# nwihardjo/SpaghettiSearch

Measured on AMD Instinct MI355X. Metric: pagerank_iters_per_sec, higher is better.
Workload: dtype f64

## Files before the change

### spaghettisearch_amd/csrc/pagerank.hip

```cpp
#include "pr_device.hpp"

#include <algorithm>
#include <chrono>
#include <cmath>
#include <memory>

namespace {

__global__ void k_pr_item_ranges(WorkItem* __restrict__ work, uint32_t n_items, const uint32_t* __restrict__ in_ptr) {
    const uint32_t i = blockIdx.x * blockDim.x + threadIdx.x;
    if (i >= n_items) return;
    WorkItem w = work[i];
    switch (w.kind) {
        case V_ROWW: w.beg = in_ptr[w.row]; w.end = in_ptr[w.row + 1]; break;
        case V_SEG:
            w.beg = in_ptr[w.row] + w.count * SEGW;
            w.end = min(in_ptr[w.row + 1], w.beg + SEGW);
            break;
        case V_QUAD:
        case V_DEG: w.beg = in_ptr[w.row]; w.end = in_ptr[w.row + w.count]; break;
        default: return;
    }
    work[i] = w;
}
// ... 422 lines not shown
    if (!out) return ctx->fail(SS_ERR_INVALID, "ss_pr_create: out is NULL");
    *out = nullptr;
    if (k_topics < 1 || !n_topic) return ctx->fail(SS_ERR_INVALID, "ss_pr_create: k_topics < 1 or n_topic NULL");
    if (k_topics > MAXK) return ctx->fail(SS_ERR_UNSUPPORTED, "ss_pr_create: k_topics %d > %d per state (ss_pagerank_run splits larger K)", k_topics, MAXK);
    SS_HIP(ctx, hipSetDevice(ctx->device));
    hipStream_t st = ctx->stream;

    ss_pr* pr = new (std::nothrow) ss_pr();
    if (!pr) return ctx->fail(SS_ERR_OOM, "ss_pr_create: host OOM");
    std::unique_ptr<ss_pr> guard(pr);
    pr->g = g;
    pr->k = k_topics;
    pick_kernel(ctx, pr, k_topics, g->nd_int);
    const int GW = pr->gw;
    const bool vitems = pr->kernel != PR_STEP;
    const int GI = pr->nwave ? 8 : GW;
    const size_t n_local = g->n_local();
    if (((uint64_t)g->nd_int + 1) * GW * 8 >= (1ull << 32))
        return ctx->fail(SS_ERR_UNSUPPORTED, "ss_pr_create: contribution table of %llu rows x %d topics exceeds 4 GiB (shard the graph over more ranks)",
                         (unsigned long long)g->nd_int, GW);

    const bool trace = ctx->opt("pr.trace", 0) != 0;
    auto t_now = [] { return std::chrono::steady_clock::now(); };
    auto t_ms = [](std::chrono::steady_clock::time_point a, std::chrono::steady_clock::time_point b) { return std::chrono::duration<double, std::milli>(b - a).count(); };
    SS_HIP(ctx, pr->x.alloc(n_local * GW));
    bool share = GW >= 8 && g->world == 1 && ctx->opt("pr.affine", 0) == 0 && ctx->opt("pr.share_zero_rows", 1) != 0;
    if (!share) SS_TRY(alloc_tables(pr, st, (size_t)g->nd_int + 1));

    const auto tc0 = t_now();
    const PlanOptions opt = plan_options(ctx, pr, n_local);
    Cut cut = cut_items(g->h_indeg_nd, g->h_indeg_d, g->sl_nd, GI, pr->nwave, opt);
    const uint32_t n_tail = g->cnt_nd - cut.pos_nd;
    struct PinGuard { ss_ctx* c; void* p = nullptr; size_t cap = 0; ~PinGuard() { c->pin_free(p, cap); } } tail_od{ctx};
    if (share && n_tail == 0) {
        share = false;
        SS_TRY(alloc_tables(pr, st, (size_t)g->nd_int + 1));
    }
    if (share) {
        tail_od.p = ctx->pin_alloc((size_t)n_tail * sizeof(uint32_t), &tail_od.cap);
        if (!tail_od.p) return ctx->fail(SS_ERR_OOM, "ss_pr_create: no pinned host memory for %u out-degrees", n_tail);
        SS_HIP(ctx, hipMemcpyAsync(tail_od.p, g->outdeg.p + cut.pos_nd, (size_t)n_tail * sizeof(uint32_t), hipMemcpyDeviceToHost, st));
    }
    const auto tc1 = t_now();
    const int per_cu = blocks_per_cu(pr->kernel, GW);
    const auto tc1a = t_now();
    pr->nblocks = grid_for(ctx, pr, opt, per_cu, cut.items.size());
    static const std::vector<uint32_t> no_woff;
    const std::vector<uint32_t>* woff = &no_woff;
    if (vitems) {
        const uint32_t nw = pr->nblocks * WAVES;
        const auto td0 = t_now();
        const std::vector<double>& cost = item_costs(cut, g->h_indeg_nd, g->h_indeg_d, g->sl_nd, GI, pr->nwave);
        const auto td0a = t_now();
        std::vector<uint32_t>& owner = deal_items(cut, cost, nw, pr->nwave, opt);
#ifdef SS_PR_WAVETIME
        dump_wave_loads(cut, cost, owner, nw);
#endif
        const auto td1 = t_now();
        if (trace) fprintf(stderr, "[pr trace]   deal: occupancy query %.2f ms, costs %.3f ms, owners %.3f ms\n", t_ms(tc1, tc1a), t_ms(td0, td0a), t_ms(td0a, td1));
        woff = &place_items(cut, owner, nw);
        if (trace) fprintf(stderr, "[pr trace]   deal: placement %.3f ms\n", t_ms(td1, t_now()));
    }
    const std::vector<WorkItem>& items = cut.items;

    g->settle();
    const auto tc2 = t_now();
    SharedRows sh;
    if (share) {
        SS_HIP(ctx, hipStreamSynchronize(st));
        const auto ts0 = t_now();
        sh = plan_shared_rows(static_cast<const uint32_t*>(tail_od.p), n_tail, cut.pos_nd);
        const auto ts1 = t_now();
        SS_TRY(alloc_tables(pr, st, (size_t)sh.table_rows));
        SS_HIP(ctx, pr->sh_deg.alloc(sh.deg.size()));
        SS_HIP(ctx, hipMemcpyAsync(pr->sh_deg.p, sh.deg.data(), sh.deg.size() * sizeof(uint32_t), hipMemcpyHostToDevice, st));
        SS_HIP(ctx, pr->src_shared.alloc(g->e_local));
        if (g->e_local)
            hipLaunchKernelGGL(k_pr_remap_src, dim3((unsigned)std::min<uint64_t>(ss::div_up(g->e_local, TPB), (uint64_t)ctx->cu_count * 16)), dim3(TPB), 0, st,
                               (const uint32_t*)g->in_src.p, pr->src_shared.p, (size_t)g->e_local, cut.pos_nd, g->cnt_nd, (const uint32_t*)g->outdeg.p,
                               (const uint32_t*)pr->sh_deg.p, (uint32_t)sh.deg.size(), sh.zrow);
        if (trace) fprintf(stderr, "[pr trace]   shared rows: %u rows without in-edges -> %zu shared rows (host %.3f ms), table %llu rows\n", n_tail, sh.deg.size(),
                           t_ms(ts0, ts1), (unsigned long long)sh.table_rows);
    }
    SS_HIP(ctx, pr->partials.alloc(((size_t)std::max(pr->nblocks, ss::begin_blocks(pr)) + 8) * 2 * GW));
    SS_HIP(ctx, pr->segpart.alloc((size_t)std::max(cut.nsegs, 1u) * GW));
    SS_HIP(ctx, pr->rowticket.alloc(std::max(cut.nmulti, 1u)));
    SS_HIP(ctx, hipMemsetAsync(pr->rowticket.p, 0, pr->rowticket.bytes(), st));
    SS_HIP(ctx, pr->woff.alloc(std::max<size_t>(woff->size(), 8)));
    if (!woff->empty()) SS_HIP(ctx, hipMemcpyAsync(pr->woff.p, woff->data(), woff->size() * sizeof(uint32_t), hipMemcpyHostToDevice, st));
    SS_HIP(ctx, pr->work.alloc(items.size()));
    SS_HIP(ctx, hipMemcpyAsync(pr->work.p, items.data(), items.size() * sizeof(WorkItem), hipMemcpyHostToDevice, st));
    if (vitems)
        hipLaunchKernelGGL(k_pr_item_ranges, dim3(ss::div_up(items.size(), TPB)), dim3(TPB), 0, st, pr->work.p, (uint32_t)items.size(), (const uint32_t*)g->in_ptr.p);
    SS_HIP(ctx, pr->ctl.alloc(1));
    SS_HIP(ctx, hipMemsetAsync(pr->ctl.p, 0, sizeof(PrCtl), st));
    double h_x0[MAXK];
    for (int k = 0; k < MAXK; k++) h_x0[k] = k < k_topics ? 1.0 / (double)n_topic[k] : 0.0;
    SS_HIP(ctx, pr->x0.alloc(MAXK));
    SS_HIP(ctx, hipMemcpyAsync(pr->x0.p, h_x0, sizeof(h_x0), hipMemcpyHostToDevice, st));
    SS_HIP(ctx, hipStreamSynchronize(st));
    if (trace) fprintf(stderr, "[pr trace] ss_pr_create: build_work %.2f ms (%zu items), edge ranges + deal %.2f ms, alloc + upload %.2f ms\n", t_ms(tc0, tc1), items.size(), t_ms(tc1, tc2), t_ms(tc2, t_now()));
    if (trace) fprintf(stderr, "[pr trace] where the state lives: x %p  tab0 %p  tab1 %p  in_src %p  in_ptr %p  outdeg %p  work %p  woff %p\n", (void*)pr->x.p, (void*)pr->tab0.p,
                       (void*)pr->tab1.p, (void*)g->in_src.p, (void*)g->in_ptr.p, (void*)g->outdeg.p, (void*)pr->work.p, (void*)pr->woff.p);

    fill_params(pr, cut, opt, damping, eps, max_iter, k_topics);
    if (share) {
        PrParams& p = pr->prm;
        p.in_src = pr->src_shared.p;
        p.sh_deg = pr->sh_deg.p;
        p.n_shared = (uint32_t)sh.deg.size();
        p.share = 1;
        p.zrow = sh.zrow;
        p.tab_rows = cut.pos_nd;
    }
    if (trace) trace_plan(pr, items, *woff);
    g->users++;
    *out = guard.release();
    return SS_OK;
}

int32_t ss_pr_set_teleport(ss_pr* pr, const uint64_t* set_ptr, const uint32_t* set_nodes) {
    if (!pr) return SS_ERR_INVALID;
    ss_ctx* ctx = pr->g->ctx;
    std::lock_guard<std::recursive_mutex> lk(ctx->mu);
    SS_HIP(ctx, hipSetDevice(ctx->device));
    if (pr->begun) return ctx->fail(SS_ERR_STATE, "ss_pr_set_teleport: call before ss_pr_begin");
    hipStream_t st = ctx->stream;
    PrParams& p = pr->prm;
    if (!set_ptr) {
        p.memb = nullptr; p.tin = nullptr; p.nz_in = nullptr; p.ts_mask = 0;
        return SS_OK;
    }
    const ss_graph* g = pr->g;
    const int K = pr->k;
    SS_TRY(unshare_rows(pr, st));
    std::vector<uint64_t> h_ptr(K + 1);
    SS_HIP(ctx, ss::copy_in(ctx->stream, h_ptr.data(), set_ptr, (K + 1) * sizeof(uint64_t)));
    if (h_ptr[0] != 0) return ctx->fail(SS_ERR_INVALID, "ss_pr_set_teleport: set_ptr[0] != 0");
    for (int k = 0; k < K; k++)
        if (h_ptr[k + 1] < h_ptr[k]) return ctx->fail(SS_ERR_INVALID, "ss_pr_set_teleport: set_ptr not non-decreasing");
    const uint64_t total = h_ptr[K];
    if (total && !set_nodes) return ctx->fail(SS_ERR_INVALID, "ss_pr_set_teleport: set_nodes is NULL");
    double h_tin[MAXK];
    uint32_t mask = 0;
    for (int k = 0; k < MAXK; k++) {
        h_tin[k] = 0.0;
        if (k < K && h_ptr[k + 1] > h_ptr[k]) {
            mask |= 1u << k;
            h_tin[k] = p.teleport * (double)g->n / (double)(h_ptr[k + 1] - h_ptr[k]);
        }
    }
    const size_t n_local = g->n_local();
    ss::DevBuf<uint64_t> d_ptr;
    ss::DevBuf<uint32_t> d_nodes, d_err, d_seen;
    ss::DevBuf<unsigned long long> d_cnt;
    SS_HIP(ctx, d_ptr.alloc(K + 1));
    SS_HIP(ctx, d_seen.alloc(g->n));
    SS_HIP(ctx, hipMemsetAsync(d_seen.p, 0, std::max<size_t>(d_seen.bytes(), 4), st));
    SS_HIP(ctx, d_nodes.alloc(total));
    SS_HIP(ctx, d_err.alloc(1));
    SS_HIP(ctx, d_cnt.alloc(MAXK));
    SS_HIP(ctx, pr->memb.alloc(n_local));
    SS_HIP(ctx, pr->tin.alloc(MAXK));
    SS_HIP(ctx, pr->nz_in.alloc(MAXK));
    SS_HIP(ctx, hipMemcpyAsync(d_ptr.p, h_ptr.data(), (K + 1) * sizeof(uint64_t), hipMemcpyHostToDevice, st));
    if (total) SS_HIP(ctx, hipMemcpyAsync(d_nodes.p, set_nodes, total * sizeof(uint32_t), hipMemcpyDefault, st));
    SS_HIP(ctx, hipMemsetAsync(pr->memb.p, 0, std::max<size_t>(pr->memb.bytes(), 4), st));
// ... 245 lines not shown
```

### spaghettisearch_amd/csrc/pr_device.hpp

```cpp
#pragma once
#include "pr_state.hpp"

#include <cmath>

namespace {


template <int GW>
__device__ __forceinline__ double wave_sum_topic(double v) {
#pragma unroll
    for (int off = GW; off < 64; off <<= 1) v += __shfl_xor(v, off, 64);
    return v;
}

__device__ __forceinline__ double zero_row_rank(const PrParams& p, int sweep, double S, double x0) {
    return ((sweep == 0 ? x0 : 0.0) + p.teleport) / S;
}
__device__ __forceinline__ double teleport_of(const PrParams& p, uint32_t lrow, int t) {
    if (!p.memb || !((p.ts_mask >> t) & 1u)) return p.teleport;
    return ((p.memb[lrow] >> t) & 1u) ? p.tin[t] : 0.0;
}
__device__ __forceinline__ double zero_row_rank_ts(const PrParams& p, int sweep, double S, double x0, double tele) {
    return ((sweep == 0 ? x0 : 0.0) + tele) / S;
}

template <int PS, typename T>
__device__ __forceinline__ T ctl_ld(const T* q) {
    if constexpr (PS) return __hip_atomic_load(q, __ATOMIC_RELAXED, __HIP_MEMORY_SCOPE_AGENT);
    else return *q;
}
template <int PS, typename T>
__device__ __forceinline__ void ctl_st(T* q, T v) {
    if constexpr (PS) __hip_atomic_store(q, v, __ATOMIC_RELAXED, __HIP_MEMORY_SCOPE_AGENT);
    else *q = v;
}

template <int PS = 0>
__device__ __forceinline__ void finalize_ctl(const PrParams& p, const double* dl, const double* cs, bool is_begin) {
    PrCtl* ctl = p.ctl;
    if (p.aff) {
        AffCtl* a = p.aff;
        if (is_begin) {
            const double r1 = cs[0], s1 = cs[1] + p.tele_n, sigma = r1 + s1;
            for (int k = 0; k < MAXK; k++) {
                const bool real = k < 2;
                ctl->xz[k] = real ? p.x0[k] : 0.0;
                ctl->xz_in[k] = ctl->xz[k];
                ctl->S[k] = real ? sigma : 1.0;
                ctl->csum[k] = real ? cs[k] : 0.0;
                ctl->delta[k] = 0.0;
                ctl->active[k] = real ? 1 : 0;
                ctl->iters[k] = 0;
                ctl->tele[k] = 0.0;
            }
            ctl->tele[1] = p.teleport;
            a->r_x = 0.0; a->s_x = 1.0;
            a->r_prev = 0.0; a->s_prev = 1.0;
            a->r_next = r1 / sigma; a->s_next = s1 / sigma;
            a->xz_prev[0] = ctl->xz[0];
            a->xz_prev[1] = ctl->xz[1];
            a->it = 0;
            ctl->sweep = 0;
            ctl->n_active = 2;
            return;
        }
        const int it = ctl->sweep + 1;
        a->r_prev = a->r_x; a->s_prev = a->s_x;
        a->r_x = a->r_next; a->s_x = a->s_next;
        for (int k = 0; k < 2; k++) {
            a->xz_prev[k] = ctl->xz[k];
            ctl->xz[k] = zero_row_rank_ts(p, ctl->sweep, ctl->S[k], p.x0[k], ctl->tele[k]);
            ctl->xz_in[k] = ctl->xz[k];
            ctl->iters[k] = it;
            ctl->csum[k] = cs[k];
        }
        const double r1 = cs[0] + p.tele_n * a->r_x;
        const double s1 = cs[1] + p.tele_n * a->s_x;
        const double sigma = r1 + s1;
        a->r_next = r1 / sigma;
        a->s_next = s1 / sigma;
        ctl->tele[0] = p.teleport * a->r_x;
        ctl->tele[1] = p.teleport * a->s_x;
        ctl->S[0] = ctl->S[1] = sigma;
        ctl->sweep = it;
        return;
    }
    if (is_begin) {
        for (int k = 0; k < MAXK; k++) {
            const bool real = k < p.k_topics;
            ctl->xz[k] = real ? p.x0[k] : 0.0;
            ctl->xz_in[k] = real ? p.x0[k] : 0.0;
            ctl->S[k] = real ? cs[k] + p.tele_n : 1.0;
            ctl->csum[k] = real ? cs[k] : 0.0;
            ctl->delta[k] = 0.0;
            ctl->active[k] = real ? 1 : 0;
            ctl->iters[k] = 0;
        }
        ctl->sweep = 0;
        ctl->n_active = p.k_topics;
        return;
    }
    const int sw = ctl_ld<PS>(&ctl->sweep);
    const int it = sw + 1;
    int na = 0;
    for (int k = 0; k < p.k_topics; k++) {
        if (ctl_ld<PS>(&ctl->active[k])) {
            const double Sk = ctl_ld<PS>(&ctl->S[k]);
            ctl_st<PS>(&ctl->iters[k], it);
            ctl_st<PS>(&ctl->delta[k], dl[k]);
            if (p.memb && ((p.ts_mask >> k) & 1u)) {
                ctl_st<PS>(&ctl->xz[k], zero_row_rank_ts(p, sw, Sk, p.x0[k], 0.0));
                ctl_st<PS>(&ctl->xz_in[k], zero_row_rank_ts(p, sw, Sk, p.x0[k], p.tin[k]));
            } else {
                const double xz = zero_row_rank(p, sw, Sk, p.x0[k]);
                ctl_st<PS>(&ctl->xz[k], xz);
                ctl_st<PS>(&ctl->xz_in[k], xz);
            }
            bool cont = dl[k] > p.eps;
            if (p.max_iter > 0 && it >= p.max_iter) cont = false;
            ctl_st<PS>(&ctl->active[k], cont ? 1 : 0);
            na += cont ? 1 : 0;
            ctl_st<PS>(&ctl->S[k], cs[k] + p.tele_n);
            ctl_st<PS>(&ctl->csum[k], cs[k]);
        }
    }
    ctl_st<PS>(&ctl->n_active, na);
    if constexpr (PS) {
        asm volatile("s_waitcnt vmcnt(0)" ::: "memory");
    }
    ctl_st<PS>(&ctl->sweep, it);
}

template <int GW, int PS = 0>
__device__ __forceinline__ void block_reduce_and_publish(const PrParams& p, double dsum, double csum, double* tail,
                                                         bool is_begin) {
    __shared__ double red[WAVES][2][MAXK];
    __shared__ double tot[2][MAXK];
    __shared__ double colsum[TPB];
    __shared__ int s_last;
    const int lane = threadIdx.x & 63, wave = threadIdx.x >> 6;
    const int t = lane % GW;
    dsum = wave_sum_topic<GW>(dsum);
    csum = wave_sum_topic<GW>(csum);
    if (lane < GW) {
        red[wave][0][t] = dsum;
        red[wave][1][t] = csum;
    }
    __syncthreads();
    if (threadIdx.x < 2 * GW) {
        const int which = threadIdx.x / GW, tt = threadIdx.x % GW;
        double v = red[0][which][tt];
#pragma unroll
        for (int w = 1; w < WAVES; w++) v += red[w][which][tt];
        __hip_atomic_store(&p.partials[(size_t)blockIdx.x * 2 * GW + threadIdx.x], v, __ATOMIC_RELAXED, __HIP_MEMORY_SCOPE_AGENT);
    }
    asm volatile("s_waitcnt vmcnt(0)" ::: "memory");
    __syncthreads();
    constexpr unsigned NG = 8;
    constexpr int NCOL = 2 * GW;
    constexpr int NPART = TPB / NCOL;
    const unsigned ng = min(NG, gridDim.x);
    const unsigned grp = blockIdx.x % ng;
    const unsigned members = (gridDim.x - grp + ng - 1) / ng;
    double* const gpart = p.partials + (size_t)gridDim.x * NCOL;
    if (threadIdx.x == 0) {
        if constexpr (PS == 2) {
            __builtin_amdgcn_fence(__ATOMIC_RELEASE, "agent");
            asm volatile("s_waitcnt vmcnt(0)" ::: "memory");
        }
        const unsigned prev = __hip_atomic_fetch_add(&p.ctl->gticket[grp], 1u, __ATOMIC_RELAXED, __HIP_MEMORY_SCOPE_AGENT);
        s_last = prev == members - 1;
    }
    __syncthreads();
    if (!s_last) return;
    const int col = threadIdx.x % NCOL, part = threadIdx.x / NCOL;
    {
        double acc = 0.0;
        for (unsigned m0 = part; m0 < members; m0 += 16 * NPART) {
            double v[16];
#pragma unroll
            for (int u = 0; u < 16; u++) {
                const unsigned m = m0 + u * NPART;
                v[u] = __hip_atomic_load(&p.partials[(size_t)(grp + ng * (m < members ? m : m0)) * NCOL + col], __ATOMIC_RELAXED, __HIP_MEMORY_SCOPE_AGENT);
            }
#pragma unroll
            for (int u = 0; u < 16; u++)
                if (m0 + u * NPART < members) acc += v[u];
        }
        colsum[threadIdx.x] = acc;
    }
    __syncthreads();
    if (threadIdx.x < NCOL) {
        double v = 0.0;
        for (int q = 0; q < NPART; q++) v += colsum[q * NCOL + threadIdx.x];
        __hip_atomic_store(&gpart[(size_t)grp * NCOL + threadIdx.x], v, __ATOMIC_RELAXED, __HIP_MEMORY_SCOPE_AGENT);
    }
    if (threadIdx.x == 0) ctl_st<PS>(&p.ctl->gticket[grp], 0u);
    asm volatile("s_waitcnt vmcnt(0)" ::: "memory");
    __syncthreads();
    if (threadIdx.x == 0) {
        const unsigned prev = __hip_atomic_fetch_add(&p.ctl->ticket, 1u, __ATOMIC_RELAXED, __HIP_MEMORY_SCOPE_AGENT);
        s_last = prev == ng - 1;
    }
    __syncthreads();
    if (!s_last) return;
    if (threadIdx.x < NCOL) {
        double v = 0.0;
        for (unsigned gq = 0; gq < ng; gq++)
            v += __hip_atomic_load(&gpart[(size_t)gq * NCOL + threadIdx.x], __ATOMIC_RELAXED, __HIP_MEMORY_SCOPE_AGENT);
        tot[threadIdx.x / GW][threadIdx.x % GW] = v;
    }
    __syncthreads();
    if (!is_begin && threadIdx.x < GW && ctl_ld<PS>(&p.ctl->active[threadIdx.x])) {
        const double n_zero = (double)((p.cnt_nd - p.pos_nd) + (p.cnt_d - p.pos_d));
        if (p.memb && ((p.ts_mask >> threadIdx.x) & 1u)) {
            const int k = threadIdx.x;
            const double out_new = zero_row_rank_ts(p, ctl_ld<PS>(&p.ctl->sweep), ctl_ld<PS>(&p.ctl->S[k]), p.x0[k], 0.0);
            const double in_new = zero_row_rank_ts(p, ctl_ld<PS>(&p.ctl->sweep), ctl_ld<PS>(&p.ctl->S[k]), p.x0[k], p.tin[k]);
            tot[0][k] += (n_zero - p.nz_in[k]) * fabs(out_new - ctl_ld<PS>(&p.ctl->xz[k])) + p.nz_in[k] * fabs(in_new - ctl_ld<PS>(&p.ctl->xz_in[k]));
        } else {
            const double xz_new = zero_row_rank(p, ctl_ld<PS>(&p.ctl->sweep), ctl_ld<PS>(&p.ctl->S[threadIdx.x]), p.x0[threadIdx.x]);
            tot[0][threadIdx.x] += n_zero * fabs(xz_new - ctl_ld<PS>(&p.ctl->xz[threadIdx.x]));
        }
    }
    __syncthreads();
    if (p.world == 1) {
        if (threadIdx.x == 0) {
            double dl[MAXK], cs[MAXK];
            for (int k = 0; k < MAXK; k++) {
                dl[k] = k < GW ? tot[0][k] : 0.0;
                cs[k] = k < GW ? tot[1][k] : 0.0;
            }
            ctl_st<PS>(&p.ctl->ticket, 0u);
            finalize_ctl<PS>(p, dl, cs, is_begin);
        }
    } else {
        if (threadIdx.x < GW) {
            tail[(size_t)(p.sl_nd - 2) * GW + threadIdx.x] = tot[1][threadIdx.x];
            tail[(size_t)(p.sl_nd - 1) * GW + threadIdx.x] = tot[0][threadIdx.x];
        }
        if (threadIdx.x == 0) p.ctl->ticket = 0;
    }
}

template <int GA, int GB>
__device__ __attribute__((used, noinline)) void begin_caller_context(const PrParams& p, double* tail) {
    if (!__builtin_constant_p(p.world)) return;
    block_reduce_and_publish<GA>(p, 0.0, 0.0, tail, true);
    block_reduce_and_publish<GB>(p, 0.0, 0.0, tail, true);
}

#define NT_LOAD(p) __builtin_nontemporal_load(p)
#define NT_STORE(v, p) __builtin_nontemporal_store(v, p)

constexpr uint32_t SRC_MASK = 0x7FFFFFFFu;

}
```

### spaghettisearch_amd/csrc/pr_state.hpp

```cpp
#pragma once
#include "graph.hpp"
#include "pr_plan.hpp"

#ifdef SS_PR_WAVETIME
#include <cstdio>
#include <cstdlib>
#include <string>
#endif

namespace {

constexpr int MAXK = 16;

struct PrCtl {
    double S[MAXK];
    double delta[MAXK];
    double csum[MAXK];
    double xz[MAXK];
    double xz_in[MAXK];
    double tele[MAXK];
    int32_t active[MAXK];
    int32_t iters[MAXK];
    int32_t sweep;
    int32_t n_active;
    uint32_t ticket;
    uint32_t stuck;
    uint32_t gticket[8];
};

constexpr int AFF_MAXK = 256;
constexpr unsigned AFF_NB = 512;
struct AffCtl {
    double u[AFF_MAXK];
    double delta[AFF_MAXK];
    int32_t active[AFF_MAXK], iters[AFF_MAXK], just[AFF_MAXK];
    double r_x, r_prev, r_next;
    double s_x, s_prev, s_next;
    double xz_prev[2];
    int32_t n_active, n_just, k_real, it;
};

struct PrParams {
    const uint32_t* in_ptr;
    const uint32_t* in_src;
    const uint32_t* outdeg;
    double* x;
    const double* tab_rd[2];
    double* tab_wr[2];
    const WorkItem* work;
    double* partials;
    double* segpart;
    uint32_t* rowticket;
    PrCtl* ctl;
    const double* x0;
    double d, teleport, eps, tele_n;
    int32_t max_iter, k_topics, world;
    uint32_t sl_nd, cnt_nd, sl_d, cnt_d, seg_edges, n_items;
    uint32_t pos_nd, pos_d;
    const uint32_t* memb;
    const double* tin;
    const double* nz_in;
    uint32_t ts_mask;
    uint32_t zrow;
    const uint32_t* woff;
    uint32_t stagger_div;
    uint32_t stagger_code;
    uint32_t class_order;
    uint32_t n_order;
    double* x_alt;
    AffCtl* aff;
    const double* tele_col;
    const uint32_t* sh_deg;
    uint32_t n_shared;
    uint32_t share;
    uint32_t tab_rows;
};

}

enum PrKernel : int {
    PR_STEP = 0,
    PR_SWEEP = 1,
    PR_SWEEP_N = 2,
};

struct ss_pr {
    ss_graph* g = nullptr;
    PrKernel kernel = PR_SWEEP;
    int gw = 1;
    ss::DevBuf<float> wire_send, wire_recv;
    bool nwave = false;
    int persist_mode = 1;
    bool persist = false;
    int k = 1;
    PrParams prm{};
    unsigned nblocks = 0;
    ss::DevBuf<double> x, tab0, tab1, send, partials, segpart, x0;
    ss::DevBuf<uint32_t> rowticket;
    ss::DevBuf<uint32_t> memb;
    ss::DevBuf<double> tin, nz_in;
    ss::DevBuf<WorkItem> work;
    ss::DevBuf<uint32_t> woff;
    ss::DevBuf<uint32_t> src_shared;
    ss::DevBuf<uint32_t> sh_deg;
    ss::DevBuf<PrCtl> ctl;
    bool begun = false;
    bool need_finalize = false;
    bool finalize_is_begin = false;
};

// ... 41 lines not shown
```

### spaghettisearch_amd/csrc/pr_sweep.hip

```cpp
#include "pr_device.hpp"

#include <algorithm>

namespace {

template <int GW>
__device__ __forceinline__ double tab_at(const double* __restrict__ T, uint32_t row, int t) {
    return *reinterpret_cast<const double*>(reinterpret_cast<const char*>(T) + (size_t)((row * (uint32_t)GW + (uint32_t)t) * 8u));
}


template <int GW, bool TS>
struct SweepCtx {
    const PrParams& p;
    const double* __restrict__ T;
    double* __restrict__ Tw;
    double S, x0;
    bool act;
    int t, gbase, slot;
    double dsum, csum;
};

__device__ __forceinline__ uint32_t turn_fill(uint32_t epos, uint32_t lim) {
    return min((uint32_t)CH, __builtin_elementwise_sub_sat(lim, epos));
// ... 150 lines not shown
        for (int j = 0; j < CH; j++) acc += v[j];
        if (ends) {
            const uint32_t od = (uint32_t)__shfl((int)co, c.gbase + (int)q, 64);
            if (valid) finish_row<GW>(c, lrow, acc, xo, od);
            acc = 0.0;
        }
        q = qn;
        ch = cn;
        if (cross) {
            it++;
            cur = nxt;
            cb = nb; ce = ne; co = no;
            nq = (cur.count + NS - 1) / NS;
            nch = cur.nseg;
            nxt = work[it + 1];
            bounds(nxt, it + 1 < i1, nb, ne, no);
        }
    }
}

template <int GW, int R, bool TS>
__device__ __forceinline__ void deg_rows(SweepCtx<GW, TS>& c, const WorkItem* __restrict__ work, uint32_t i0, uint32_t i1) {
    constexpr int NS = 64 / GW;
    constexpr int DM = CH / R;
    constexpr int IR = CH / GW;
    const PrParams& p = c.p;
    if (i0 >= i1) return;
    auto idx = [&](const WorkItem& w, bool live, uint32_t turn, uint32_t (&src)[IR]) __attribute__((always_inline)) {
        const uint32_t rb = (turn * NS + (uint32_t)c.slot) * R;
#pragma unroll
        for (int r = 0; r < IR; r++) {
            const uint32_t j = (uint32_t)(r * GW + c.t);
            const uint32_t rr = rb + j / DM, u = j % DM;
            const bool ok = live && u < w.nseg && rr < w.count;
            const uint32_t raw = NT_LOAD(&p.in_src[ok ? w.beg + rr * w.nseg + u : 0u]);
            src[r] = ok ? (raw & SRC_MASK) : p.zrow;
        }
    };
    WorkItem cur = work[i0], nxt = work[i0 + 1];
    uint32_t src_n[IR];
    idx(cur, true, 0, src_n);
    for (uint32_t it = i0; it < i1; it++) {
        const WorkItem nn = work[it + 2];
        const uint32_t row0 = cur.row, count = cur.count;
        const uint32_t turns = (count + NS * R - 1) / (NS * R);
        for (uint32_t i = 0; i < turns; i++) {
            uint32_t src[IR];
#pragma unroll
            for (int r = 0; r < IR; r++) src[r] = src_n[r];
            if (i + 1 < turns) idx(cur, true, i + 1, src_n);
            else idx(nxt, it + 1 < i1, 0, src_n);
            const uint32_t rb = (i * NS + (uint32_t)c.slot) * R;
            double xo[R];
#pragma unroll
            for (int r = 0; r < R; r++) xo[r] = NT_LOAD(&p.x[(size_t)(row0 + (rb + r < count ? rb + r : 0u)) * GW + c.t]);
            const uint32_t myr = row0 + (rb + (uint32_t)c.t < count ? rb + (uint32_t)c.t : 0u);
            const uint32_t odv = (c.t < R && myr < p.sl_nd) ? NT_LOAD(&p.outdeg[myr]) : 1u;
            double v[CH];
            gather_turn<GW>(c.T, src, c.t, c.gbase, v);
#pragma unroll
            for (int r = 0; r < R; r++) {
                double y = 0.0;
#pragma unroll
                for (int u = 0; u < DM; u++) y += v[r * DM + u];
                const uint32_t od = (uint32_t)__shfl((int)odv, c.gbase + r, 64);
                if (rb + r < count) finish_row<GW>(c, row0 + rb + r, y, xo[r], od);
            }
        }
        cur = nxt;
        nxt = nn;
    }
}

#ifndef SS_PR_MINW
#define SS_PR_MINW 1
#endif
#ifdef SS_PR_WAVETIME
__device__ unsigned long long g_pr_wt[65536][2];
#endif
template <int GW, bool TS>
__global__ __launch_bounds__(TPB, SS_PR_MINW) void k_pr_sweep(PrParams p) {
    constexpr int NS = 64 / GW;
    PrCtl* ctl = p.ctl;
    if (ctl->n_active == 0) return;
#ifdef SS_PR_WAVETIME
    unsigned long long wt0;
    asm volatile("s_memrealtime %0\n\ts_waitcnt lgkmcnt(0)" : "=s"(wt0));
#endif
    const int sweep = ctl->sweep;
    const int lane = threadIdx.x & 63;
    const uint32_t wave = (uint32_t)__builtin_amdgcn_readfirstlane((int)(threadIdx.x >> 6));
    SweepCtx<GW, TS> c{p, p.tab_rd[sweep & 1], p.tab_wr[sweep & 1], 0.0, 0.0, false, lane % GW, lane - lane % GW, lane / GW, 0.0, 0.0};
    c.S = ctl->S[c.t];
    c.act = ctl->active[c.t] != 0;
    c.x0 = sweep == 0 ? p.x0[c.t] : 0.0;

    if constexpr (!TS) {
        if (p.n_shared) {
            const double xz_out = c.act ? zero_row_rank(p, sweep, c.S, p.x0[c.t]) : ctl->xz[c.t];
            const uint32_t nel = p.n_shared * (uint32_t)GW;
            for (uint32_t i = blockIdx.x * TPB + threadIdx.x; i < nel; i += gridDim.x * TPB)
                c.Tw[(size_t)(p.zrow + 1) * GW + i] = p.d * xz_out / (double)p.sh_deg[i / GW];
        }
    }

    const uint32_t* __restrict__ off = p.woff + (size_t)(blockIdx.x * WAVES + wave) * 8;
    int rot = p.stagger_div ? (int)((blockIdx.x / p.stagger_div) % 6u) : 0;
    if (p.stagger_code) {
        uint32_t cdv = p.stagger_code;
        for (uint32_t r = blockIdx.x / p.stagger_div; r > 0; r--) cdv /= 6u;
        rot = (int)(cdv % 6u);
    }
    for (int s6 = 0; s6 < 6; s6++) {
    const int cls = (int)((p.class_order >> (3 * ((s6 + rot) % 6))) & 7u);
    {
        int ln = lane;
        asm volatile("" : "+v"(ln));
        c.t = ln % GW;
        c.gbase = ln - ln % GW;
        c.slot = ln / GW;
    }
    switch (cls) {
    case 0: long_rows<GW>(c, p.work, off[0], off[1], lane); break;
    case 1: quad_rows<GW>(c, p.work, off[1], off[2]); break;
    case 2: deg_rows<GW, 2>(c, p.work, off[2], off[3]); break;
    case 3: deg_rows<GW, 4>(c, p.work, off[3], off[4]); break;
    case 4: deg_rows<GW, 8>(c, p.work, off[4], off[5]); break;
    default:
    for (uint32_t item = off[5]; item < off[6]; item++) {
        const WorkItem w = p.work[item];
        const bool store = TS || !p.share;
        const bool ts = TS && p.memb && ((p.ts_mask >> c.t) & 1u);
        const double xz_out = c.act ? (ts ? zero_row_rank_ts(p, sweep, c.S, p.x0[c.t], 0.0) : zero_row_rank(p, sweep, c.S, p.x0[c.t])) : ctl->xz[c.t];
        const double xz_inn = ts ? (c.act ? zero_row_rank_ts(p, sweep, c.S, p.x0[c.t], p.tin[c.t]) : ctl->xz_in[c.t]) : xz_out;
        uint32_t od[16];
#pragma unroll
        for (int i = 0; i < 16; i++) {
            const uint32_t rr = (uint32_t)(i * NS + c.slot);
            od[i] = NT_LOAD(&p.outdeg[w.row + (rr < w.count ? rr : 0u)]);
        }
#pragma unroll
        for (int i = 0; i < 16; i++) {
            const uint32_t rr = (uint32_t)(i * NS + c.slot);
            if (rr < w.count) {
                const uint32_t lrow = w.row + rr;
                const double xz = ts && ((p.memb[lrow] >> c.t) & 1u) ? xz_inn : xz_out;
                const double cc = p.d * xz / (double)od[i];
                if (store) NT_STORE(cc, &c.Tw[(size_t)lrow * GW + c.t]);
                c.csum += cc;
            }
        }
    }
    break;
    }
    }
#ifdef SS_PR_WAVETIME
    {
        unsigned long long wt1;
        asm volatile("s_waitcnt vmcnt(0)\n\ts_memrealtime %0\n\ts_waitcnt lgkmcnt(0)" : "=s"(wt1));
        const uint32_t wid = (blockIdx.x * WAVES + wave) & 65535u;
        if (lane == 0) { g_pr_wt[wid][0] = wt0; g_pr_wt[wid][1] = wt1; }
    }
#endif
    block_reduce_and_publish<GW>(p, c.dsum, c.csum, c.Tw, false);
}

template __device__ void begin_caller_context<8, 16>(const PrParams&, double*);

}

namespace ss {
void pr_sweep_launch(ss_pr* pr, hipStream_t st) {
    const bool ts = pr->prm.memb != nullptr;
    if (pr->gw == 8) {
        if (ts) hipLaunchKernelGGL((k_pr_sweep<8, true>), dim3(pr->nblocks), dim3(TPB), 0, st, pr->prm);
        else hipLaunchKernelGGL((k_pr_sweep<8, false>), dim3(pr->nblocks), dim3(TPB), 0, st, pr->prm);
    } else {
        if (ts) hipLaunchKernelGGL((k_pr_sweep<16, true>), dim3(pr->nblocks), dim3(TPB), 0, st, pr->prm);
        else hipLaunchKernelGGL((k_pr_sweep<16, false>), dim3(pr->nblocks), dim3(TPB), 0, st, pr->prm);
    }
}
int pr_sweep_occupancy(int gw) {
    int per_cu = 8;
    if (gw == 8) (void)hipOccupancyMaxActiveBlocksPerMultiprocessor(&per_cu, k_pr_sweep<8, false>, TPB, 0);
    else (void)hipOccupancyMaxActiveBlocksPerMultiprocessor(&per_cu, k_pr_sweep<16, false>, TPB, 0);
    return per_cu;
}

#ifdef SS_PR_WAVETIME
void pr_dump_wave_times(const ss_pr* pr) {
    if (pr->gw < 8) return;
    (void)hipDeviceSynchronize();
    const uint32_t nwv = std::min<uint32_t>(65536u, pr->nblocks * WAVES);
    std::vector<unsigned long long> h((size_t)nwv * 2);
    if (hipMemcpyFromSymbol(h.data(), HIP_SYMBOL(g_pr_wt), h.size() * sizeof(unsigned long long)) != hipSuccess || !nwv) return;
    unsigned long long t0 = ~0ull;
    for (uint32_t w = 0; w < nwv; w++) t0 = std::min(t0, h[2 * w]);
    std::vector<double> st(nwv), en(nwv);
    for (uint32_t w = 0; w < nwv; w++) { st[w] = (double)(h[2 * w] - t0) / 100.0; en[w] = (double)(h[2 * w + 1] - t0) / 100.0; }
    std::sort(st.begin(), st.end()); std::sort(en.begin(), en.end());
    if (FILE* f = open_dump("pr_wt.csv")) {
        fprintf(f, "wave,start_us,end_us\n");
        for (uint32_t w = 0; w < nwv; w++) fprintf(f, "%u,%.2f,%.2f\n", w, (double)(h[2 * w] - t0) / 100.0, (double)(h[2 * w + 1] - t0) / 100.0);
        fclose(f);
    }
    fprintf(stderr, "[pr wavetime] %u waves: start us median %.1f max %.1f | out of items us min %.1f p10 %.1f median %.1f p90 %.1f p99 %.1f max %.1f\n", nwv,
            st[nwv / 2], st[nwv - 1], en[0], en[nwv / 10], en[nwv / 2], en[nwv * 9 / 10], en[(size_t)nwv * 99 / 100], en[nwv - 1]);
}
#endif
}
```

### spaghettisearch_amd/csrc/pr_sweep_n.hip

```cpp
#include "pr_device.hpp"

namespace {

#ifndef SS_PRN_MINW
#define SS_PRN_MINW 6
#endif
template <int KW>
struct NVec { double v[KW]; };
template <int KW, int PS = 0>
__device__ __forceinline__ NVec<KW> ntab(const double* __restrict__ T, uint32_t row) {
    NVec<KW> r;
    if constexpr (PS == 1) {
        const double* q = reinterpret_cast<const double*>(reinterpret_cast<const char*>(T) + (size_t)(row * (8u * KW)));
#pragma unroll
        for (int k = 0; k < KW; k++) r.v[k] = __hip_atomic_load(q + k, __ATOMIC_RELAXED, __HIP_MEMORY_SCOPE_AGENT);
    } else if constexpr (KW == 1) {
        r.v[0] = *reinterpret_cast<const double*>(reinterpret_cast<const char*>(T) + (size_t)(row * 8u));
    } else {
        const double2 t = *reinterpret_cast<const double2*>(reinterpret_cast<const char*>(T) + (size_t)(row * 16u));
        r.v[0] = t.x;
        r.v[1] = t.y;
    }
    return r;
}
// ... 187 lines not shown
    #pragma unroll
                        for (int u = 0; u < 4; u++) {
                            const uint32_t j = b + ch * 16u + (uint32_t)(u * 8 + gl);
                            const uint32_t raw = NT_LOAD(&in_src[j < e_end ? j : b]);
                            src[u] = j < e_end ? (raw & SRC_MASK) : p.zrow;
                        }
                    };
                    idx32(0, src_n);
                    for (uint32_t ch = 0; ch < w.nseg; ch += 2) {
                        uint32_t src[4];
    #pragma unroll
                        for (int u = 0; u < 4; u++) src[u] = src_n[u];
                        idx32(ch + 2, src_n);
                        NVec<KW> v[4];
    #pragma unroll
                        for (int u = 0; u < 4; u++) v[u] = ntab<KW, PS>(c.T, src[u]);
    #pragma unroll
                        for (int u = 0; u < 4; u++)
    #pragma unroll
                            for (int k = 0; k < KW; k++) acc.v[k] += v[u].v[k];
                    }
    #pragma unroll
                    for (int k = 0; k < KW; k++)
    #pragma unroll
                        for (int o = 1; o < 8; o <<= 1) acc.v[k] += __shfl_xor(acc.v[k], o, 64);
                    if (valid && gl == 0) finish_n<KW, TS, PS>(c, lrow, acc, xo, od);
                }
            }
        }

    } break;
    case 2: {
        for (uint32_t it = off[2]; it < off[5]; it++) {
            const WorkItem w = p.work[it];
            if (w.nseg <= 2) deg_lane_rows<KW, TS, 2, PS>(c, w, lane);
            else if (w.nseg <= 4) deg_lane_rows<KW, TS, 4, PS>(c, w, lane);
            else deg_lane_rows<KW, TS, 8, PS>(c, w, lane);
        }

    } break;
    default: {
        for (uint32_t it = off[5]; it < off[6]; it++) {
            const WorkItem w = p.work[it];
            for (uint32_t r0 = 0; r0 < w.count; r0 += 64) {
                const uint32_t rr = r0 + (uint32_t)lane;
                if (rr >= w.count) continue;
                const uint32_t lrow = w.row + rr;
                const uint32_t od = NT_LOAD(&p.outdeg[lrow]);
    #pragma unroll
                for (int k = 0; k < KW; k++) {
                    const bool ts = TS && p.memb && ((p.ts_mask >> k) & 1u);
                    const double xz_out = c.act[k] ? (ts ? zero_row_rank_ts(p, sweep, c.S[k], p.x0[k], 0.0) : zero_row_rank_ts(p, sweep, c.S[k], p.x0[k], c.tele[k])) : ctl_ld<PS>(&ctl->xz[k]);
                    const double xz_inn = ts ? (c.act[k] ? zero_row_rank_ts(p, sweep, c.S[k], p.x0[k], p.tin[k]) : ctl_ld<PS>(&ctl->xz_in[k])) : xz_out;
                    const double xz = ts && ((p.memb[lrow] >> k) & 1u) ? xz_inn : xz_out;
                    const double cc = p.d * xz / (double)od;
                    tab_store<PS>(cc, &c.Tw[(size_t)lrow * KW + k]);
                    c.csum[k] += cc;
                }
            }
        }

    } break;
    }
    }

    double ds = c.dsum[0], cs = c.csum[0];
    if constexpr (KW == 2) {
        const double d0o = __shfl_xor(c.dsum[0], 1, 64), d1o = __shfl_xor(c.dsum[1], 1, 64);
        const double c0o = __shfl_xor(c.csum[0], 1, 64), c1o = __shfl_xor(c.csum[1], 1, 64);
        ds = (lane & 1) ? c.dsum[1] + d1o : c.dsum[0] + d0o;
        cs = (lane & 1) ? c.csum[1] + c1o : c.csum[0] + c0o;
    }
    block_reduce_and_publish<KW, PS>(p, ds, cs, c.Tw, false);
}

template <int KW, bool TS>
__global__ __launch_bounds__(TPB, SS_PRN_MINW) void k_pr_sweep_n(PrParams p) {
    const PrCtl* ctl = p.ctl;
    const int n_active = ctl->n_active, sweep = ctl->sweep;
    double S_in[KW];
    int act_in[KW];
#pragma unroll
    for (int k = 0; k < KW; k++) { S_in[k] = ctl->S[k]; act_in[k] = ctl->active[k]; }
    if (n_active == 0) return;
    sweep_n_body<KW, TS, false>(p, sweep, S_in, act_in);
}

constexpr uint32_t MULTI_SPIN_MAX = 1u << 24;
template <int KW, int PSM>
__global__ __launch_bounds__(TPB, SS_PRN_MINW) void k_pr_multi_n(PrParams p, int n_steps) {
    __shared__ int s_go, s_na, s_sw, s_act[KW];
    __shared__ double s_S[KW];
    PrCtl* ctl = p.ctl;
    auto read_ctl = [&]() __attribute__((always_inline)) {
        s_na = ctl_ld<1>(&ctl->n_active) == 0 || ctl_ld<1>(&ctl->stuck) ? 0 : 1;
        s_sw = ctl_ld<1>(&ctl->sweep);
#pragma unroll
        for (int k = 0; k < KW; k++) { s_S[k] = ctl_ld<1>(&ctl->S[k]); s_act[k] = ctl_ld<1>(&ctl->active[k]); }
    };
    if (threadIdx.x == 0) read_ctl();
    __syncthreads();
    for (int s = 0; s < n_steps; s++) {
        if (s_na == 0) return;
        const int sweep = s_sw;
        double S_in[KW];
        int act_in[KW];
#pragma unroll
        for (int k = 0; k < KW; k++) { S_in[k] = s_S[k]; act_in[k] = s_act[k]; }
        __syncthreads();
        sweep_n_body<KW, false, PSM>(p, sweep, S_in, act_in);
        if (s + 1 == n_steps) return;
        if (threadIdx.x == 0) {
            uint32_t spins = 0;
            while (ctl_ld<1>(&ctl->sweep) == sweep && ++spins < MULTI_SPIN_MAX) __builtin_amdgcn_s_sleep(8);
            const bool ok = spins < MULTI_SPIN_MAX;
            if (!ok) ctl_st<1>(&ctl->stuck, 1u);
            s_go = ok ? 1 : 0;
            if (ok) read_ctl();
            if constexpr (PSM == 2) {
                __builtin_amdgcn_fence(__ATOMIC_ACQUIRE, "agent");
                asm volatile("s_waitcnt vmcnt(0)" ::: "memory");
            }
        }
        __syncthreads();
        if (!s_go) return;
    }
}

template __device__ void begin_caller_context<1, 2>(const PrParams&, double*);

}

namespace ss {
void pr_sweep_n_launch(ss_pr* pr, hipStream_t st) {
    const bool ts = pr->prm.memb != nullptr;
    if (pr->gw == 1) {
        if (ts) hipLaunchKernelGGL((k_pr_sweep_n<1, true>), dim3(pr->nblocks), dim3(TPB), 0, st, pr->prm);
        else hipLaunchKernelGGL((k_pr_sweep_n<1, false>), dim3(pr->nblocks), dim3(TPB), 0, st, pr->prm);
    } else {
        if (ts) hipLaunchKernelGGL((k_pr_sweep_n<2, true>), dim3(pr->nblocks), dim3(TPB), 0, st, pr->prm);
        else hipLaunchKernelGGL((k_pr_sweep_n<2, false>), dim3(pr->nblocks), dim3(TPB), 0, st, pr->prm);
    }
}
int pr_sweep_n_occupancy(int gw) {
    int per_cu = 8;
    if (gw == 1) (void)hipOccupancyMaxActiveBlocksPerMultiprocessor(&per_cu, k_pr_sweep_n<1, false>, TPB, 0);
    else (void)hipOccupancyMaxActiveBlocksPerMultiprocessor(&per_cu, k_pr_sweep_n<2, false>, TPB, 0);
    return per_cu;
}
void pr_multi_n_launch(ss_pr* pr, hipStream_t st, int n_steps) {
    if (pr->gw == 1) {
        if (pr->persist_mode == 2) hipLaunchKernelGGL((k_pr_multi_n<1, 2>), dim3(pr->nblocks), dim3(TPB), 0, st, pr->prm, n_steps);
        else hipLaunchKernelGGL((k_pr_multi_n<1, 1>), dim3(pr->nblocks), dim3(TPB), 0, st, pr->prm, n_steps);
    } else {
        if (pr->persist_mode == 2) hipLaunchKernelGGL((k_pr_multi_n<2, 2>), dim3(pr->nblocks), dim3(TPB), 0, st, pr->prm, n_steps);
        else hipLaunchKernelGGL((k_pr_multi_n<2, 1>), dim3(pr->nblocks), dim3(TPB), 0, st, pr->prm, n_steps);
    }
}
int pr_multi_n_occupancy(int gw) {
    int per_cu = 0;
    if (gw == 1) (void)hipOccupancyMaxActiveBlocksPerMultiprocessor(&per_cu, k_pr_multi_n<1, 1>, TPB, 0);
    else (void)hipOccupancyMaxActiveBlocksPerMultiprocessor(&per_cu, k_pr_multi_n<2, 1>, TPB, 0);
    return per_cu;
}
}
```

Baseline: 18500.

## Flatten grid reduction to single ticket, wave-parallel finalize, prefetch first work item

Replaces the two-level grouped ticket reduction with a single global ticket: the last block sums all partials itself, grouped by eight interleaved slots, which removes the second atomic round and the per-group publish. Control finalization is spread across a wave so that each lane handles one topic, with a ballot for the active count, instead of a serial loop on thread 0. The sweep kernels hoist the control and offset loads ahead of the early exit and warm the first work item and its in-edge sources before the main loop, to hide launch latency. PrCtl is reordered so the hot fields sit together. The last block now does more serial load work, and the ticket reset moves into finalize.

Result: no change. 18480 (median of 2 runs) (-0.1%).

```diff
diff --git a/spaghettisearch_amd/csrc/pagerank.hip b/spaghettisearch_amd/csrc/pagerank.hip
--- a/spaghettisearch_amd/csrc/pagerank.hip
+++ b/spaghettisearch_amd/csrc/pagerank.hip
@@ -528,7 +528,7 @@
         if (trace) fprintf(stderr, "[pr trace]   shared rows: %u rows without in-edges -> %zu shared rows (host %.3f ms), table %llu rows\n", n_tail, sh.deg.size(),
                            t_ms(ts0, ts1), (unsigned long long)sh.table_rows);
     }
-    SS_HIP(ctx, pr->partials.alloc(((size_t)std::max(pr->nblocks, ss::begin_blocks(pr)) + 8) * 2 * GW));
+    SS_HIP(ctx, pr->partials.alloc((size_t)std::max(pr->nblocks, ss::begin_blocks(pr)) * 2 * GW));
     SS_HIP(ctx, pr->segpart.alloc((size_t)std::max(cut.nsegs, 1u) * GW));
     SS_HIP(ctx, pr->rowticket.alloc(std::max(cut.nmulti, 1u)));
     SS_HIP(ctx, hipMemsetAsync(pr->rowticket.p, 0, pr->rowticket.bytes(), st));
diff --git a/spaghettisearch_amd/csrc/pr_device.hpp b/spaghettisearch_amd/csrc/pr_device.hpp
--- a/spaghettisearch_amd/csrc/pr_device.hpp
+++ b/spaghettisearch_amd/csrc/pr_device.hpp
@@ -4,6 +4,22 @@
 #include <cmath>
 
 namespace {
+
+#define NT_LOAD(p) __builtin_nontemporal_load(p)
+#define NT_STORE(v, p) __builtin_nontemporal_store(v, p)
+
+constexpr uint32_t SRC_MASK = 0x7FFFFFFFu;
+
+
+__device__ __forceinline__ void warm_first_item(const PrParams& p, uint32_t i0, uint32_t i1, int lane, uint32_t stride) {
+    if (i0 >= i1) return;
+    const WorkItem cur = p.work[i0], nxt = p.work[i0 + 1];
+    asm volatile("" ::"s"(nxt.kind));
+    if (cur.end > cur.beg) {
+        const uint32_t w = NT_LOAD(&p.in_src[min(cur.beg + (uint32_t)lane * stride, cur.end - 1u)]);
+        asm volatile("" ::"v"(w));
+    }
+}
 
 
 template <int GW>
@@ -131,12 +147,47 @@
     ctl_st<PS>(&ctl->sweep, it);
 }
 
+template <int PS>
+__device__ __forceinline__ void finalize_ctl_wave(const PrParams& p, double (*tot)[MAXK], int lane) {
+    PrCtl* ctl = p.ctl;
+    const int sw = ctl_ld<PS>(&ctl->sweep);
+    const int it = sw + 1;
+    bool cont = false;
+    if (lane < p.k_topics && ctl_ld<PS>(&ctl->active[lane])) {
+        const int k = lane;
+        const double dlk = tot[0][k], csk = tot[1][k];
+        const double Sk = ctl_ld<PS>(&ctl->S[k]);
+        ctl_st<PS>(&ctl->iters[k], it);
+        ctl_st<PS>(&ctl->delta[k], dlk);
+        if (p.memb && ((p.ts_mask >> k) & 1u)) {
+            ctl_st<PS>(&ctl->xz[k], zero_row_rank_ts(p, sw, Sk, p.x0[k], 0.0));
+            ctl_st<PS>(&ctl->xz_in[k], zero_row_rank_ts(p, sw, Sk, p.x0[k], p.tin[k]));
+        } else {
+            const double xz = zero_row_rank(p, sw, Sk, p.x0[k]);
+            ctl_st<PS>(&ctl->xz[k], xz);
+            ctl_st<PS>(&ctl->xz_in[k], xz);
+        }
+        cont = dlk > p.eps;
+        if (p.max_iter > 0 && it >= p.max_iter) cont = false;
+        ctl_st<PS>(&ctl->active[k], cont ? 1 : 0);
+        ctl_st<PS>(&ctl->S[k], csk + p.tele_n);
+        ctl_st<PS>(&ctl->csum[k], csk);
+    }
+    const int na = __popcll(__ballot(cont));
+    if (lane == 0) ctl_st<PS>(&ctl->n_active, na);
+    if constexpr (PS) {
+        asm volatile("s_waitcnt vmcnt(0)" ::: "memory");
+    }
+    if (lane == 0) ctl_st<PS>(&ctl->sweep, it);
+}
+
 template <int GW, int PS = 0>
 __device__ __forceinline__ void block_reduce_and_publish(const PrParams& p, double dsum, double csum, double* tail,
                                                          bool is_begin) {
     __shared__ double red[WAVES][2][MAXK];
     __shared__ double tot[2][MAXK];
-    __shared__ double colsum[TPB];
+    __shared__ double colsum[4][TPB];
+    __shared__ double grow[8][2 * MAXK];
     __shared__ int s_last;
     const int lane = threadIdx.x & 63, wave = threadIdx.x >> 6;
     const int t = lane % GW;
@@ -159,56 +210,58 @@
     constexpr unsigned NG = 8;
     constexpr int NCOL = 2 * GW;
     constexpr int NPART = TPB / NCOL;
-    const unsigned ng = min(NG, gridDim.x);
-    const unsigned grp = blockIdx.x % ng;
-    const unsigned members = (gridDim.x - grp + ng - 1) / ng;
-    double* const gpart = p.partials + (size_t)gridDim.x * NCOL;
+    constexpr int U = GW >= 8 ? 4 : 1;
     if (threadIdx.x == 0) {
         if constexpr (PS == 2) {
             __builtin_amdgcn_fence(__ATOMIC_RELEASE, "agent");
             asm volatile("s_waitcnt vmcnt(0)" ::: "memory");
         }
-        const unsigned prev = __hip_atomic_fetch_add(&p.ctl->gticket[grp], 1u, __ATOMIC_RELAXED, __HIP_MEMORY_SCOPE_AGENT);
-        s_last = prev == members - 1;
+        const unsigned prev = __hip_atomic_fetch_add(&p.ctl->ticket, 1u, __ATOMIC_RELAXED, __HIP_MEMORY_SCOPE_AGENT);
+        s_last = prev == gridDim.x - 1;
     }
     __syncthreads();
     if (!s_last) return;
-    const int col = threadIdx.x % NCOL, part = threadIdx.x / NCOL;
-    {
-        double acc = 0.0;
-        for (unsigned m0 = part; m0 < members; m0 += 16 * NPART) {
-            double v[16];
-#pragma unroll
-            for (int u = 0; u < 16; u++) {
-                const unsigned m = m0 + u * NPART;
-                v[u] = __hip_atomic_load(&p.partials[(size_t)(grp + ng * (m < members ? m : m0)) * NCOL + col], __ATOMIC_RELAXED, __HIP_MEMORY_SCOPE_AGENT);
-            }
-#pragma unroll
-            for (int u = 0; u < 16; u++)
-                if (m0 + u * NPART < members) acc += v[u];
-        }
-        colsum[threadIdx.x] = acc;
-    }
-    __syncthreads();
+    const unsigned ng = min(NG, gridDim.x);
+    const unsigned col = threadIdx.x % NCOL, part = threadIdx.x / NCOL;
+    double acc[NG];
+#pragma unroll
+    for (unsigned g = 0; g < NG; g++) acc[g] = 0.0;
+    for (unsigned m0 = part; m0 * ng < gridDim.x; m0 += U * NPART) {
+        double v[NG][U];
+#pragma unroll
+        for (unsigned g = 0; g < NG; g++)
+#pragma unroll
+            for (int u = 0; u < U; u++) {
+                const unsigned b = g + ng * (m0 + (unsigned)u * NPART);
+                const bool ok = g < ng && b < gridDim.x;
+                v[g][u] = __hip_atomic_load(&p.partials[(size_t)(ok ? b : 0u) * NCOL + col], __ATOMIC_RELAXED, __HIP_MEMORY_SCOPE_AGENT);
+            }
+#pragma unroll
+        for (unsigned g = 0; g < NG; g++)
+#pragma unroll
+            for (int u = 0; u < U; u++)
+                if (g < ng && g + ng * (m0 + (unsigned)u * NPART) < gridDim.x) acc[g] += v[g][u];
+    }
+    constexpr unsigned GH = NG / 2;
+#pragma unroll
+    for (unsigned h = 0; h < NG; h += GH) {
+        if (h < ng) {
+#pragma unroll
+            for (unsigned g = 0; g < GH; g++) colsum[g][threadIdx.x] = acc[h + g];
+            __syncthreads();
+            const unsigned g = threadIdx.x / NCOL;
+            if (g < GH && h + g < ng) {
+                double v = 0.0;
+                for (int q = 0; q < NPART; q++) v += colsum[g][q * NCOL + col];
+                grow[h + g][col] = v;
+            }
+            __syncthreads();
+        }
+    }
     if (threadIdx.x < NCOL) {
-        double v = 0.0;
-        for (int q = 0; q < NPART; q++) v += colsum[q * NCOL + threadIdx.x];
-        __hip_atomic_store(&gpart[(size_t)grp * NCOL + threadIdx.x], v, __ATOMIC_RELAXED, __HIP_MEMORY_SCOPE_AGENT);
-    }
-    if (threadIdx.x == 0) ctl_st<PS>(&p.ctl->gticket[grp], 0u);
-    asm volatile("s_waitcnt vmcnt(0)" ::: "memory");
-    __syncthreads();
-    if (threadIdx.x == 0) {
-        const unsigned prev = __hip_atomic_fetch_add(&p.ctl->ticket, 1u, __ATOMIC_RELAXED, __HIP_MEMORY_SCOPE_AGENT);
-        s_last = prev == ng - 1;
-    }
-    __syncthreads();
-    if (!s_last) return;
-    if (threadIdx.x < NCOL) {
-        double v = 0.0;
-        for (unsigned gq = 0; gq < ng; gq++)
-            v += __hip_atomic_load(&gpart[(size_t)gq * NCOL + threadIdx.x], __ATOMIC_RELAXED, __HIP_MEMORY_SCOPE_AGENT);
-        tot[threadIdx.x / GW][threadIdx.x % GW] = v;
+        double total = 0.0;
+        for (unsigned g = 0; g < ng; g++) total += grow[g][threadIdx.x];
+        tot[threadIdx.x / GW][threadIdx.x % GW] = total;
     }
     __syncthreads();
     if (!is_begin && threadIdx.x < GW && ctl_ld<PS>(&p.ctl->active[threadIdx.x])) {
@@ -225,7 +278,10 @@
     }
     __syncthreads();
     if (p.world == 1) {
-        if (threadIdx.x == 0) {
+        if (!is_begin && !p.aff) {
+            if (threadIdx.x == 0) ctl_st<PS>(&p.ctl->ticket, 0u);
+            if (threadIdx.x < 64) finalize_ctl_wave<PS>(p, tot, (int)threadIdx.x);
+        } else if (threadIdx.x == 0) {
             double dl[MAXK], cs[MAXK];
             for (int k = 0; k < MAXK; k++) {
                 dl[k] = k < GW ? tot[0][k] : 0.0;
@@ -250,9 +306,4 @@
     block_reduce_and_publish<GB>(p, 0.0, 0.0, tail, true);
 }
 
-#define NT_LOAD(p) __builtin_nontemporal_load(p)
-#define NT_STORE(v, p) __builtin_nontemporal_store(v, p)
-
-constexpr uint32_t SRC_MASK = 0x7FFFFFFFu;
-
-}
+}
diff --git a/spaghettisearch_amd/csrc/pr_state.hpp b/spaghettisearch_amd/csrc/pr_state.hpp
--- a/spaghettisearch_amd/csrc/pr_state.hpp
+++ b/spaghettisearch_amd/csrc/pr_state.hpp
@@ -13,19 +13,18 @@
 constexpr int MAXK = 16;
 
 struct PrCtl {
+    int32_t sweep;
+    int32_t n_active;
+    int32_t active[MAXK];
     double S[MAXK];
     double delta[MAXK];
     double csum[MAXK];
     double xz[MAXK];
     double xz_in[MAXK];
     double tele[MAXK];
-    int32_t active[MAXK];
     int32_t iters[MAXK];
-    int32_t sweep;
-    int32_t n_active;
     uint32_t ticket;
     uint32_t stuck;
-    uint32_t gticket[8];
 };
 
 constexpr int AFF_MAXK = 256;
diff --git a/spaghettisearch_amd/csrc/pr_sweep.hip b/spaghettisearch_amd/csrc/pr_sweep.hip
--- a/spaghettisearch_amd/csrc/pr_sweep.hip
+++ b/spaghettisearch_amd/csrc/pr_sweep.hip
@@ -256,18 +256,46 @@
 __global__ __launch_bounds__(TPB, SS_PR_MINW) void k_pr_sweep(PrParams p) {
     constexpr int NS = 64 / GW;
     PrCtl* ctl = p.ctl;
-    if (ctl->n_active == 0) return;
+    const int lane = threadIdx.x & 63;
+    const uint32_t wave = (uint32_t)__builtin_amdgcn_readfirstlane((int)(threadIdx.x >> 6));
+    const int n_active = ctl->n_active, sweep = ctl->sweep;
+    double S_t = ctl->S[lane % GW];
+    int act_t = ctl->active[lane % GW];
+    double x0_t = p.x0[lane % GW];
+    const uint32_t* __restrict__ off = p.woff + (size_t)(blockIdx.x * WAVES + wave) * 8;
+    uint32_t o[7];
+#pragma unroll
+    for (int k = 0; k < 7; k++) o[k] = off[k];
+    asm volatile("" : "+s"(o[0]), "+s"(o[1]), "+s"(o[2]), "+s"(o[3]), "+s"(o[4]), "+s"(o[5]), "+s"(o[6]));
+    asm volatile("" : "+v"(S_t), "+v"(act_t), "+v"(x0_t));
+    if (n_active == 0) return;
 #ifdef SS_PR_WAVETIME
     unsigned long long wt0;
     asm volatile("s_memrealtime %0\n\ts_waitcnt lgkmcnt(0)" : "=s"(wt0));
 #endif
-    const int sweep = ctl->sweep;
-    const int lane = threadIdx.x & 63;
-    const uint32_t wave = (uint32_t)__builtin_amdgcn_readfirstlane((int)(threadIdx.x >> 6));
+    int rot = p.stagger_div ? (int)((blockIdx.x / p.stagger_div) % 6u) : 0;
+    if (p.stagger_code) {
+        uint32_t cdv = p.stagger_code;
+        for (uint32_t r = blockIdx.x / p.stagger_div; r > 0; r--) cdv /= 6u;
+        rot = (int)(cdv % 6u);
+    }
+    {
+        uint32_t f0 = 0, f1 = 0;
+        for (int s6 = 5; s6 >= 0; s6--) {
+            const int cls = (int)((p.class_order >> (3 * ((s6 + rot) % 6))) & 7u);
+            const int kc = cls < 5 ? cls : 5;
+            uint32_t a = o[0], b = o[1];
+#pragma unroll
+            for (int k = 1; k < 6; k++)
+                if (kc == k) { a = o[k]; b = o[k + 1]; }
+            if (a < b) { f0 = a; f1 = b; }
+        }
+        warm_first_item(p, f0, f1, lane, 2u);
+    }
     SweepCtx<GW, TS> c{p, p.tab_rd[sweep & 1], p.tab_wr[sweep & 1], 0.0, 0.0, false, lane % GW, lane - lane % GW, lane / GW, 0.0, 0.0};
-    c.S = ctl->S[c.t];
-    c.act = ctl->active[c.t] != 0;
-    c.x0 = sweep == 0 ? p.x0[c.t] : 0.0;
+    c.S = S_t;
+    c.act = act_t != 0;
+    c.x0 = sweep == 0 ? x0_t : 0.0;
 
     if constexpr (!TS) {
         if (p.n_shared) {
@@ -278,13 +306,6 @@
         }
     }
 
-    const uint32_t* __restrict__ off = p.woff + (size_t)(blockIdx.x * WAVES + wave) * 8;
-    int rot = p.stagger_div ? (int)((blockIdx.x / p.stagger_div) % 6u) : 0;
-    if (p.stagger_code) {
-        uint32_t cdv = p.stagger_code;
-        for (uint32_t r = blockIdx.x / p.stagger_div; r > 0; r--) cdv /= 6u;
-        rot = (int)(cdv % 6u);
-    }
     for (int s6 = 0; s6 < 6; s6++) {
     const int cls = (int)((p.class_order >> (3 * ((s6 + rot) % 6))) & 7u);
     {
@@ -295,13 +316,13 @@
         c.slot = ln / GW;
     }
     switch (cls) {
-    case 0: long_rows<GW>(c, p.work, off[0], off[1], lane); break;
-    case 1: quad_rows<GW>(c, p.work, off[1], off[2]); break;
-    case 2: deg_rows<GW, 2>(c, p.work, off[2], off[3]); break;
-    case 3: deg_rows<GW, 4>(c, p.work, off[3], off[4]); break;
-    case 4: deg_rows<GW, 8>(c, p.work, off[4], off[5]); break;
+    case 0: long_rows<GW>(c, p.work, o[0], o[1], lane); break;
+    case 1: quad_rows<GW>(c, p.work, o[1], o[2]); break;
+    case 2: deg_rows<GW, 2>(c, p.work, o[2], o[3]); break;
+    case 3: deg_rows<GW, 4>(c, p.work, o[3], o[4]); break;
+    case 4: deg_rows<GW, 8>(c, p.work, o[4], o[5]); break;
     default:
-    for (uint32_t item = off[5]; item < off[6]; item++) {
+    for (uint32_t item = o[5]; item < o[6]; item++) {
         const WorkItem w = p.work[item];
         const bool store = TS || !p.share;
         const bool ts = TS && p.memb && ((p.ts_mask >> c.t) & 1u);
diff --git a/spaghettisearch_amd/csrc/pr_sweep_n.hip b/spaghettisearch_amd/csrc/pr_sweep_n.hip
--- a/spaghettisearch_amd/csrc/pr_sweep_n.hip
+++ b/spaghettisearch_amd/csrc/pr_sweep_n.hip
@@ -293,7 +293,25 @@
     int act_in[KW];
 #pragma unroll
     for (int k = 0; k < KW; k++) { S_in[k] = ctl->S[k]; act_in[k] = ctl->active[k]; }
+    const uint32_t wave = (uint32_t)__builtin_amdgcn_readfirstlane((int)(threadIdx.x >> 6));
+    const uint32_t* __restrict__ off = p.woff + (size_t)(blockIdx.x * WAVES + wave) * 8;
+    uint32_t o[7];
+#pragma unroll
+    for (int k = 0; k < 7; k++) o[k] = off[k];
+    asm volatile("" : "+s"(o[0]), "+s"(o[1]), "+s"(o[2]), "+s"(o[3]), "+s"(o[4]), "+s"(o[5]), "+s"(o[6]));
+#pragma unroll
+    for (int k = 0; k < KW; k++) asm volatile("" : "+s"(S_in[k]), "+s"(act_in[k]));
     if (n_active == 0) return;
+    {
+        uint32_t f0 = 0, f1 = 0;
+        for (int s4 = 3; s4 >= 0; s4--) {
+            const uint32_t ph = (p.n_order >> (2 * s4)) & 3u;
+            const uint32_t a = ph == 0 ? o[0] : ph == 1 ? o[1] : ph == 2 ? o[2] : o[5];
+            const uint32_t b = ph == 0 ? o[1] : ph == 1 ? o[2] : ph == 2 ? o[5] : o[6];
+            if (a < b) { f0 = a; f1 = b; }
+        }
+        warm_first_item(p, f0, f1, (int)(threadIdx.x & 63), 8u);
+    }
     sweep_n_body<KW, TS, false>(p, sweep, S_in, act_in);
 }
 
```
